# idonahum/photoVerse

Hardware: AMD Instinct MI355X
Metric: denoising steps/sec at 512x512 bs=16, 50-step loop (2 UNet fwd + CFG + DPM-Solver++ step per step) (higher is better)
Workload: dtype f16; 1 GPU; configs[1] shape timed over 96 steps instead of 50: SD-v1.5 UNet + PhotoVerse processors, 96-step loop, bs=16/GPU, 512x512 (64x64 latents), P=1, guidance 7.5, fp16; per_gpu_batch=16, global_batch=16, latent=64, parallelism=dp1 (batch-sharded, 1 all_gather), hip_graph=True, graph_branches=2

## Files before the change

photoverse_amd/csrc/pv_rowgemm.hip:

```cpp
#include "pv_common.h"
#include <stdlib.h>

namespace {

constexpr int RG_K = 320;
constexpr int RG_CHUNK = 160;
constexpr int RG_TILE = RG_CHUNK * 128;
constexpr int RG_SLOTS = 4;
constexpr int RG_SMEM = RG_SLOTS * RG_TILE;

struct pv_rowgemm_params_dev : pv_row_gemm_params {
    uint32_t w_bytes;
};

template <int N>
__device__ __forceinline__ void rg_wait_vmcnt() {
    static_assert(N >= 0 && N < 64, "vmcnt is a 6-bit field");
    asm volatile("s_waitcnt vmcnt(%0)" ::"n"(N) : "memory");
}

template <bool GEGLU>
__global__ __launch_bounds__(256, 2) void row_gemm_kernel(const pv_rowgemm_params_dev p) {
    constexpr int C = RG_K;
    constexpr int KK = C / 32;
    constexpr int KT = C / 64;
    constexpr int NFC = RG_CHUNK / 16;
    typedef unsigned uint4_t __attribute__((ext_vector_type(4)));
    typedef unsigned uint2_t __attribute__((ext_vector_type(2)));
    extern __shared__ __attribute__((aligned(16))) char smem[];

    const int lane = pv_lane_id(), wave = pv_wave_id();
    const int fr = lane & 15, g = lane >> 4;
    const int m0 = (int)blockIdx.x * 128;
    const int rows_here = min(128, p.M - m0);
    const int n_chunks = p.N / RG_CHUNK;
    const int NT = n_chunks * KT;

    const __amdgpu_buffer_rsrc_t rw = __builtin_amdgcn_make_buffer_rsrc(const_cast<void*>(p.w), 0, (int)p.w_bytes, 0x00020000);
    const __amdgpu_buffer_rsrc_t rx = __builtin_amdgcn_make_buffer_rsrc(const_cast<half_t*>(reinterpret_cast<const half_t*>(p.x)) + (size_t)m0 * p.ld_x, 0,
                                                                        rows_here * p.ld_x * 2, 0x00020000);
    const int ld_o = p.ld_out;
    const __amdgpu_buffer_rsrc_t ro = __builtin_amdgcn_make_buffer_rsrc(reinterpret_cast<half_t*>(p.out) + (size_t)m0 * ld_o, 0, rows_here * ld_o * 2, 0x00020000);

    const int lrow = lane >> 3;
    const unsigned w_lane_off = (unsigned)lrow * (unsigned)(C * 2) + (unsigned)(((lane & 7) ^ lrow) << 4);
    const unsigned piece_off = w_lane_off + (unsigned)(wave * 8) * (unsigned)(C * 2);
    auto issue_stage = [&](int t) {
        const int nc = t / KT, kt = t - nc * KT;
        char* dst = smem + (t & (RG_SLOTS - 1)) * RG_TILE;
        const int soff = nc * RG_CHUNK * (C * 2) + kt * 128;
#pragma unroll
        for (int i = 0; i < 5; ++i)
            __builtin_amdgcn_raw_ptr_buffer_load_lds(rw, PV_LDS_PTR(dst + (wave + 4 * i) * 1024), 16, (int)piece_off, soff + i * 32 * (C * 2), 0, 0);
    };
    auto wg_barrier = [&]() {
        asm volatile("s_waitcnt lgkmcnt(0)" ::: "memory");
        __builtin_amdgcn_s_barrier();
        asm volatile("" ::: "memory");
    };

    half8_t xf[KK][2];
    int mrow[2];
#pragma unroll
    for (int qi = 0; qi < 2; ++qi) {
        mrow[qi] = wave * 32 + qi * 16 + fr;
        const int off = mrow[qi] * p.ld_x * 2 + g * 16;
#pragma unroll
        for (int kk = 0; kk < KK; ++kk) xf[kk][qi] = __builtin_bit_cast(half8_t, __builtin_amdgcn_raw_buffer_load_b128(rx, off, kk * 64, 0));
    }
    issue_stage(0);
    issue_stage(1);
    if (p.x_norm) {
        const float* tab = p.x_norm + (size_t)(m0 / p.rows_per_image) * 2 * C + g * 8;
#pragma unroll
        for (int kk = 0; kk < KK; ++kk) {
            const float4_t s0 = *reinterpret_cast<const float4_t*>(tab + kk * 32), s1 = *reinterpret_cast<const float4_t*>(tab + kk * 32 + 4);
            const float4_t h0 = *reinterpret_cast<const float4_t*>(tab + C + kk * 32), h1 = *reinterpret_cast<const float4_t*>(tab + C + kk * 32 + 4);
#pragma unroll
            for (int qi = 0; qi < 2; ++qi)
#pragma unroll
                for (int j = 0; j < 8; ++j) xf[kk][qi][j] = (half_t)((float)xf[kk][qi][j] * (j < 4 ? s0[j & 3] : s1[j & 3]) + (j < 4 ? h0[j & 3] : h1[j & 3]));
        }
    }
    if (p.ln) {
        typedef _Float16 h2_t __attribute__((ext_vector_type(2)));
        const h2_t ones = h2_t{(half_t)1.0f, (half_t)1.0f};
#pragma unroll
        for (int qi = 0; qi < 2; ++qi) {
            float sum = 0.f;
#pragma unroll
            for (int kk = 0; kk < KK; ++kk)
#pragma unroll
                for (int j = 0; j < 4; ++j) sum = __builtin_amdgcn_fdot2(h2_t{xf[kk][qi][2 * j], xf[kk][qi][2 * j + 1]}, ones, sum, false);
            const float mean = pv_quad_sum(sum) * (1.0f / (float)C);
            const half_t mh = (half_t)mean;
            const h2_t nm = h2_t{(half_t)(-mh), (half_t)(-mh)};
            float sq = 0.f;
#pragma unroll
            for (int kk = 0; kk < KK; ++kk)
#pragma unroll
                for (int j = 0; j < 4; ++j) {
                    const h2_t d = h2_t{xf[kk][qi][2 * j], xf[kk][qi][2 * j + 1]} + nm;
                    sq = __builtin_amdgcn_fdot2(d, d, sq, false);
                }
            const float dm = mean - (float)mh;
            const float var = pv_quad_sum(sq) * (1.0f / (float)C) - dm * dm;
            const float rstd = rsqrtf(fmaxf(var, 0.f) + p.ln_eps);
            const float nmr = -mean * rstd;
#pragma unroll
            for (int kk = 0; kk < KK; ++kk)
#pragma unroll
                for (int j = 0; j < 8; ++j) xf[kk][qi][j] = (half_t)fmaf((float)xf[kk][qi][j], rstd, nmr);
        }
    }
    rg_wait_vmcnt<0>();

    const int ring_lane[2] = {fr * 128 + ((g ^ (fr & 7)) << 4), fr * 128 + (((4 + g) ^ (fr & 7)) << 4)};
    const int pcol = (g & 1) ? 16 + (g - 1) * 4 : g * 4;
    constexpr int OUT_PER_CHUNK = GEGLU ? RG_CHUNK / 2 : RG_CHUNK;
    constexpr int STORES = GEGLU ? 6 : 10;

    float4_t acc[NFC][2];
    for (int it = 0; it < n_chunks / 2; ++it) {
        const int t0 = it * (2 * KT);
#pragma unroll
        for (int j = 0; j < 2 * KT; ++j) {
            const int t = t0 + j;
            const int kt = j % KT;
            const int nc = 2 * it + j / KT;
            if ((j & 1) == 0) {
                const bool stores_since = (j == 6) || (j == 0 && it > 0);
                if (t >= 2) {
                    if (stores_since) rg_wait_vmcnt<STORES>(); else rg_wait_vmcnt<0>();
                }
                wg_barrier();
                if (t + 2 < NT) issue_stage(t + 2);
                if (t + 3 < NT) issue_stage(t + 3);
            }
            if (kt == 0) {
#pragma unroll
                for (int i = 0; i < NFC; ++i)
                    acc[i][0] = acc[i][1] = p.bias ? *reinterpret_cast<const float4_t*>(p.bias + nc * RG_CHUNK + i * 16 + g * 4) : float4_t{0.f, 0.f, 0.f, 0.f};
            }
            const char* slot = smem + (t & (RG_SLOTS - 1)) * RG_TILE;
#pragma unroll
            for (int ks = 0; ks < 2; ++ks) {
                const char* base = slot + ring_lane[ks];
#pragma unroll
                for (int i = 0; i < NFC; ++i) {
                    const half8_t a = *reinterpret_cast<const half8_t*>(base + i * 2048);
#pragma unroll
                    for (int qi = 0; qi < 2; ++qi) acc[i][qi] = __builtin_amdgcn_mfma_f32_16x16x32_f16(a, xf[2 * kt + ks][qi], acc[i][qi], 0, 0, 0);
                }
            }
            if (kt == KT - 1) {
                const int ocol0 = nc * OUT_PER_CHUNK;
#pragma unroll
                for (int qi = 0; qi < 2; ++qi) {
                    const int ooff = mrow[qi] * ld_o * 2 + ocol0 * 2;
                    unsigned pk[GEGLU ? NFC / 2 : NFC][2];
                    if (GEGLU) {
#pragma unroll
                        for (int q = 0; q < NFC / 2; ++q) {
                            const float4_t v = acc[2 * q][qi], gt = acc[2 * q + 1][qi];
                            pk[q][0] = __builtin_bit_cast(unsigned, half2_t{(half_t)(v[0] * pv_gelu_erf(gt[0])), (half_t)(v[1] * pv_gelu_erf(gt[1]))});
                            pk[q][1] = __builtin_bit_cast(unsigned, half2_t{(half_t)(v[2] * pv_gelu_erf(gt[2])), (half_t)(v[3] * pv_gelu_erf(gt[3]))});
                        }
                    } else {
#pragma unroll
                        for (int i = 0; i < NFC; ++i) {
                            const float4_t v = acc[i][qi];
                            pk[i][0] = __builtin_bit_cast(unsigned, half2_t{(half_t)v[0], (half_t)v[1]});
                            pk[i][1] = __builtin_bit_cast(unsigned, half2_t{(half_t)v[2], (half_t)v[3]});
                        }
                    }
                    constexpr int NOUT = GEGLU ? NFC / 2 : NFC;
#pragma unroll
                    for (int q = 0; q < NOUT / 2; ++q) {
                        const auto v0 = __builtin_amdgcn_permlane16_swap(pk[2 * q][0], pk[2 * q + 1][0], false, false);
                        const auto v1 = __builtin_amdgcn_permlane16_swap(pk[2 * q][1], pk[2 * q + 1][1], false, false);
                        const unsigned sa0 = v0[0], sb0 = v0[1], sa1 = v1[0], sb1 = v1[1];
                        __builtin_amdgcn_raw_buffer_store_b128(uint4_t{sa0, sa1, sb0, sb1}, ro, ooff + pcol * 2 + q * 64, 0, 0);
                        asm volatile("s_nop 1" ::: "memory");
                    }
                    if (NOUT & 1)
                        __builtin_amdgcn_raw_buffer_store_b64(uint2_t{pk[NOUT - 1][0], pk[NOUT - 1][1]}, ro, ooff + g * 8 + (NOUT - 1) * 32, 0, 0);
                }
                __builtin_amdgcn_sched_barrier(0);
            }
        }
    }
}

}

extern "C" int pv_row_gemm(const pv_row_gemm_params* pp, void* stream) {
    pv_rowgemm_params_dev p;
    static_cast<pv_row_gemm_params&>(p) = *pp;
    if (!p.x || !p.w || !p.out || p.M <= 0 || p.K != RG_K || p.N <= 0 || (p.N % (2 * RG_CHUNK)) || (p.ld_x % 8) || (p.ld_out % 8) || p.ld_x < RG_K ||
        p.ld_out < (p.geglu ? p.N / 2 : p.N) || (p.x_norm && (p.ln || p.rows_per_image <= 0 || (p.rows_per_image % 128) || (p.M % p.rows_per_image))))
        return (int)hipErrorInvalidValue;
    if ((size_t)p.N * RG_K * 2 >= (1ull << 31)) return (int)hipErrorInvalidValue;
    p.w_bytes = (uint32_t)p.N * RG_K * 2;
    static bool attr_set_dev[64][2] = {};
    int dev_id = 0;
    (void)hipGetDevice(&dev_id);
    bool& attr_set = attr_set_dev[dev_id & 63][p.geglu ? 1 : 0];
    auto kern = p.geglu ? row_gemm_kernel<true> : row_gemm_kernel<false>;
    if (!attr_set) {
        hipError_t e = hipFuncSetAttribute(reinterpret_cast<const void*>(kern), hipFuncAttributeMaxDynamicSharedMemorySize, RG_SMEM);
        if (e != hipSuccess) return (int)e;
        attr_set = true;
    }
    hipLaunchKernelGGL(kern, dim3((unsigned)((p.M + 127) / 128)), dim3(256), RG_SMEM, (hipStream_t)stream, p);
    return PV_CHECK_LAUNCH();
}
```

Baseline: 33.31 denoising steps/s (bs=16 per GPU, summed over GPUs).

## Split row-GEMM N-chunk into two row groups and interleave epilogue with MFMA stages

Restructures the row GEMM pipeline so each 160-column weight chunk is split into a 96-row and a 64-row group, streamed through a 6-slot LDS ring in stage pairs. The epilogue (GELU/pack/store) of one group is spread across the MFMA stages of the other group using sched_group_barrier pacing, so the stores and transcendental work overlap matrix math. Bias loads move to buffer loads issued ahead of use, and the vmcnt waits are recomputed per stage. This hides epilogue and store latency, at the cost of much more complex scheduling code and the risk of wrong vmcnt accounting or extra register pressure.

```diff
diff --git a/photoverse_amd/csrc/pv_rowgemm.hip b/photoverse_amd/csrc/pv_rowgemm.hip
--- a/photoverse_amd/csrc/pv_rowgemm.hip
+++ b/photoverse_amd/csrc/pv_rowgemm.hip
@@ -1,13 +1,16 @@
 #include "pv_common.h"
 #include <stdlib.h>
+#include <type_traits>
 
 namespace {
 
 constexpr int RG_K = 320;
 constexpr int RG_CHUNK = 160;
-constexpr int RG_TILE = RG_CHUNK * 128;
-constexpr int RG_SLOTS = 4;
-constexpr int RG_SMEM = RG_SLOTS * RG_TILE;
+constexpr int RG_ROWS_A = 96;
+constexpr int RG_SLOT = RG_ROWS_A * 128;
+constexpr int RG_SLOTS = 6;
+constexpr int RG_PAIRS = 5;
+constexpr int RG_SMEM = RG_SLOTS * RG_SLOT;
 
 struct pv_rowgemm_params_dev : pv_row_gemm_params {
     uint32_t w_bytes;
@@ -25,6 +28,7 @@
     constexpr int KK = C / 32;
     constexpr int KT = C / 64;
     constexpr int NFC = RG_CHUNK / 16;
+    constexpr int NFA = RG_ROWS_A / 16, NFB = NFC - NFA;
     typedef unsigned uint4_t __attribute__((ext_vector_type(4)));
     typedef unsigned uint2_t __attribute__((ext_vector_type(2)));
     extern __shared__ __attribute__((aligned(16))) char smem[];
@@ -34,24 +38,28 @@
     const int m0 = (int)blockIdx.x * 128;
     const int rows_here = min(128, p.M - m0);
     const int n_chunks = p.N / RG_CHUNK;
-    const int NT = n_chunks * KT;
 
     const __amdgpu_buffer_rsrc_t rw = __builtin_amdgcn_make_buffer_rsrc(const_cast<void*>(p.w), 0, (int)p.w_bytes, 0x00020000);
     const __amdgpu_buffer_rsrc_t rx = __builtin_amdgcn_make_buffer_rsrc(const_cast<half_t*>(reinterpret_cast<const half_t*>(p.x)) + (size_t)m0 * p.ld_x, 0,
                                                                         rows_here * p.ld_x * 2, 0x00020000);
+    const __amdgpu_buffer_rsrc_t rb = __builtin_amdgcn_make_buffer_rsrc(const_cast<float*>(p.bias), 0, p.bias ? p.N * 4 : 0, 0x00020000);
     const int ld_o = p.ld_out;
     const __amdgpu_buffer_rsrc_t ro = __builtin_amdgcn_make_buffer_rsrc(reinterpret_cast<half_t*>(p.out) + (size_t)m0 * ld_o, 0, rows_here * ld_o * 2, 0x00020000);
 
     const int lrow = lane >> 3;
     const unsigned w_lane_off = (unsigned)lrow * (unsigned)(C * 2) + (unsigned)(((lane & 7) ^ lrow) << 4);
     const unsigned piece_off = w_lane_off + (unsigned)(wave * 8) * (unsigned)(C * 2);
-    auto issue_stage = [&](int t) {
-        const int nc = t / KT, kt = t - nc * KT;
-        char* dst = smem + (t & (RG_SLOTS - 1)) * RG_TILE;
-        const int soff = nc * RG_CHUNK * (C * 2) + kt * 128;
-#pragma unroll
-        for (int i = 0; i < 5; ++i)
-            __builtin_amdgcn_raw_ptr_buffer_load_lds(rw, PV_LDS_PTR(dst + (wave + 4 * i) * 1024), 16, (int)piece_off, soff + i * 32 * (C * 2), 0, 0);
+    auto issue_pair = [&](int c, int pp, int sp) {
+#pragma unroll
+        for (int h = 0; h < 2; ++h) {
+            const int j = 2 * pp + h, grp = j >= KT ? 1 : 0, kt = j - grp * KT;
+            char* dst = smem + (2 * sp + h) * RG_SLOT;
+            const int soff = (c * RG_CHUNK + grp * RG_ROWS_A) * (C * 2) + kt * 128;
+#pragma unroll
+            for (int i = 0; i < 3; ++i)
+                if (i < (grp ? 2 : 3))
+                    __builtin_amdgcn_raw_ptr_buffer_load_lds(rw, PV_LDS_PTR(dst + (wave + 4 * i) * 1024), 16, (int)piece_off, soff + i * 32 * (C * 2), 0, 0);
+        }
     };
     auto wg_barrier = [&]() {
         asm volatile("s_waitcnt lgkmcnt(0)" ::: "memory");
@@ -68,8 +76,8 @@
 #pragma unroll
         for (int kk = 0; kk < KK; ++kk) xf[kk][qi] = __builtin_bit_cast(half8_t, __builtin_amdgcn_raw_buffer_load_b128(rx, off, kk * 64, 0));
     }
-    issue_stage(0);
-    issue_stage(1);
+    issue_pair(0, 0, 0);
+    issue_pair(0, 1, 1);
     if (p.x_norm) {
         const float* tab = p.x_norm + (size_t)(m0 / p.rows_per_image) * 2 * C + g * 8;
 #pragma unroll
@@ -113,83 +121,125 @@
                 for (int j = 0; j < 8; ++j) xf[kk][qi][j] = (half_t)fmaf((float)xf[kk][qi][j], rstd, nmr);
         }
     }
-    rg_wait_vmcnt<0>();
 
     const int ring_lane[2] = {fr * 128 + ((g ^ (fr & 7)) << 4), fr * 128 + (((4 + g) ^ (fr & 7)) << 4)};
     const int pcol = (g & 1) ? 16 + (g - 1) * 4 : g * 4;
     constexpr int OUT_PER_CHUNK = GEGLU ? RG_CHUNK / 2 : RG_CHUNK;
-    constexpr int STORES = GEGLU ? 6 : 10;
 
     float4_t acc[NFC][2];
-    for (int it = 0; it < n_chunks / 2; ++it) {
-        const int t0 = it * (2 * KT);
-#pragma unroll
-        for (int j = 0; j < 2 * KT; ++j) {
-            const int t = t0 + j;
-            const int kt = j % KT;
-            const int nc = 2 * it + j / KT;
-            if ((j & 1) == 0) {
-                const bool stores_since = (j == 6) || (j == 0 && it > 0);
-                if (t >= 2) {
-                    if (stores_since) rg_wait_vmcnt<STORES>(); else rg_wait_vmcnt<0>();
-                }
-                wg_barrier();
-                if (t + 2 < NT) issue_stage(t + 2);
-                if (t + 3 < NT) issue_stage(t + 3);
+    float4_t bz[NFA];
+    unsigned pk[2 * NFA];
+
+    auto load_bias = [&](int c, int fb, int nf) {
+#pragma unroll
+        for (int i = 0; i < NFA; ++i)
+            if (i < nf) bz[i] = __builtin_bit_cast(float4_t, __builtin_amdgcn_raw_buffer_load_b128(rb, g * 16, (c * RG_CHUNK + (fb + i) * 16) * 4, 0));
+    };
+
+    auto epi_word = [&](auto grp_tag, int h, int c) {
+        constexpr int GRP = decltype(grp_tag)::value, NFG = GRP ? NFB : NFA, FB = GRP ? NFA : 0;
+        constexpr int NW = GEGLU ? NFG : 2 * NFG, NOF = NW / 2;
+        const int qi = h / NW, w = h % NW, ql = w >> 1, hf = w & 1;
+        if (GEGLU) {
+            const float4_t v = acc[FB + 2 * ql][qi], gt = acc[FB + 2 * ql + 1][qi];
+            pk[w] = __builtin_bit_cast(unsigned, half2_t{(half_t)(v[2 * hf] * pv_gelu_erf(gt[2 * hf])), (half_t)(v[2 * hf + 1] * pv_gelu_erf(gt[2 * hf + 1]))});
+        } else {
+            const float4_t v = acc[FB + ql][qi];
+            pk[w] = __builtin_bit_cast(unsigned, half2_t{(half_t)v[2 * hf], (half_t)v[2 * hf + 1]});
+        }
+        if (w == NW - 1) {
+            const int ooff = mrow[qi] * ld_o * 2 + (c * OUT_PER_CHUNK + FB * (GEGLU ? 8 : 16)) * 2;
+#pragma unroll
+            for (int q = 0; q < NOF / 2; ++q) {
+                const auto v0 = __builtin_amdgcn_permlane16_swap(pk[4 * q], pk[4 * q + 2], false, false);
+                const auto v1 = __builtin_amdgcn_permlane16_swap(pk[4 * q + 1], pk[4 * q + 3], false, false);
+                const unsigned sa0 = v0[0], sb0 = v0[1], sa1 = v1[0], sb1 = v1[1];
+                __builtin_amdgcn_raw_buffer_store_b128(uint4_t{sa0, sa1, sb0, sb1}, ro, ooff + pcol * 2 + q * 64, 0, 0);
+                asm volatile("s_nop 1" ::: "memory");
             }
-            if (kt == 0) {
-#pragma unroll
-                for (int i = 0; i < NFC; ++i)
-                    acc[i][0] = acc[i][1] = p.bias ? *reinterpret_cast<const float4_t*>(p.bias + nc * RG_CHUNK + i * 16 + g * 4) : float4_t{0.f, 0.f, 0.f, 0.f};
+            if (NOF & 1) __builtin_amdgcn_raw_buffer_store_b64(uint2_t{pk[2 * (NOF - 1)], pk[2 * (NOF - 1) + 1]}, ro, ooff + g * 8 + (NOF - 1) * 32, 0, 0);
+        }
+    };
+
+    auto stage = [&](auto j_tag, auto epi_tag, int c, int sp) {
+        constexpr int j = decltype(j_tag)::value;
+        constexpr bool EPI = decltype(epi_tag)::value;
+        constexpr int GRP = j >= KT ? 1 : 0, kt = j - GRP * KT, NFG = GRP ? NFB : NFA, FB = GRP ? NFA : 0;
+        if (kt == 0) {
+#pragma unroll
+            for (int i = 0; i < NFG; ++i) acc[FB + i][0] = acc[FB + i][1] = bz[i];
+        }
+        const char* slot = smem + (2 * sp + (j & 1)) * RG_SLOT;
+#pragma unroll
+        for (int ks = 0; ks < 2; ++ks) {
+            const char* base = slot + ring_lane[ks];
+#pragma unroll
+            for (int i = 0; i < NFG; ++i) {
+                const half8_t a = *reinterpret_cast<const half8_t*>(base + i * 2048);
+#pragma unroll
+                for (int qi = 0; qi < 2; ++qi) acc[FB + i][qi] = __builtin_amdgcn_mfma_f32_16x16x32_f16(a, xf[2 * kt + ks][qi], acc[FB + i][qi], 0, 0, 0);
             }
-            const char* slot = smem + (t & (RG_SLOTS - 1)) * RG_TILE;
-#pragma unroll
-            for (int ks = 0; ks < 2; ++ks) {
-                const char* base = slot + ring_lane[ks];
-#pragma unroll
-                for (int i = 0; i < NFC; ++i) {
-                    const half8_t a = *reinterpret_cast<const half8_t*>(base + i * 2048);
-#pragma unroll
-                    for (int qi = 0; qi < 2; ++qi) acc[i][qi] = __builtin_amdgcn_mfma_f32_16x16x32_f16(a, xf[2 * kt + ks][qi], acc[i][qi], 0, 0, 0);
-                }
-            }
-            if (kt == KT - 1) {
-                const int ocol0 = nc * OUT_PER_CHUNK;
-#pragma unroll
-                for (int qi = 0; qi < 2; ++qi) {
-                    const int ooff = mrow[qi] * ld_o * 2 + ocol0 * 2;
-                    unsigned pk[GEGLU ? NFC / 2 : NFC][2];
-                    if (GEGLU) {
-#pragma unroll
-                        for (int q = 0; q < NFC / 2; ++q) {
-                            const float4_t v = acc[2 * q][qi], gt = acc[2 * q + 1][qi];
-                            pk[q][0] = __builtin_bit_cast(unsigned, half2_t{(half_t)(v[0] * pv_gelu_erf(gt[0])), (half_t)(v[1] * pv_gelu_erf(gt[1]))});
-                            pk[q][1] = __builtin_bit_cast(unsigned, half2_t{(half_t)(v[2] * pv_gelu_erf(gt[2])), (half_t)(v[3] * pv_gelu_erf(gt[3]))});
-                        }
-                    } else {
-#pragma unroll
-                        for (int i = 0; i < NFC; ++i) {
-                            const float4_t v = acc[i][qi];
-                            pk[i][0] = __builtin_bit_cast(unsigned, half2_t{(half_t)v[0], (half_t)v[1]});
-                            pk[i][1] = __builtin_bit_cast(unsigned, half2_t{(half_t)v[2], (half_t)v[3]});
-                        }
-                    }
-                    constexpr int NOUT = GEGLU ? NFC / 2 : NFC;
-#pragma unroll
-                    for (int q = 0; q < NOUT / 2; ++q) {
-                        const auto v0 = __builtin_amdgcn_permlane16_swap(pk[2 * q][0], pk[2 * q + 1][0], false, false);
-                        const auto v1 = __builtin_amdgcn_permlane16_swap(pk[2 * q][1], pk[2 * q + 1][1], false, false);
-                        const unsigned sa0 = v0[0], sb0 = v0[1], sa1 = v1[0], sb1 = v1[1];
-                        __builtin_amdgcn_raw_buffer_store_b128(uint4_t{sa0, sa1, sb0, sb1}, ro, ooff + pcol * 2 + q * 64, 0, 0);
-                        asm volatile("s_nop 1" ::: "memory");
-                    }
-                    if (NOUT & 1)
-                        __builtin_amdgcn_raw_buffer_store_b64(uint2_t{pk[NOUT - 1][0], pk[NOUT - 1][1]}, ro, ooff + g * 8 + (NOUT - 1) * 32, 0, 0);
-                }
-                __builtin_amdgcn_sched_barrier(0);
-            }
-        }
-    }
+        }
+        constexpr int NM = 4 * NFG;
+        constexpr int NFO = GRP ? NFA : NFB, H = 2 * (GEGLU ? NFO : 2 * NFO);
+        constexpr int lo = kt * H / KT, hi = (kt + 1) * H / KT;
+        static_assert(2 * H / KT <= H / 2 - 1 && H / 2 - 1 < 3 * H / KT && 4 * H / KT <= H - 1, "epilogue stores must fall into stages 2 and 4");
+        if (EPI) {
+            const int ce = GRP ? c : c - 1;
+#pragma unroll
+            for (int h = lo; h < hi; ++h) epi_word(std::integral_constant<int, 1 - GRP>{}, h, ce);
+        }
+        constexpr bool PACE_VALU = EPI && GEGLU;
+        constexpr int NT = PACE_VALU ? 4 * (hi - lo) : 0;
+        constexpr int NV = (kt == 0 ? 8 * NFG : 0) + (PACE_VALU ? 19 * (hi - lo) + 8 : 0);
+        static_assert(NT <= NM, "at most one transcendental per MFMA");
+        __builtin_amdgcn_sched_group_barrier(0x100, NFG, 0);
+#pragma unroll
+        for (int m = 0; m < NM; ++m) {
+            if (NV) __builtin_amdgcn_sched_group_barrier(0x002, (NV + NM - 1) / NM, 0);
+            if ((m + 1) * NT / NM != m * NT / NM) __builtin_amdgcn_sched_group_barrier(0x400, 1, 0);
+            __builtin_amdgcn_sched_group_barrier(0x008, 1, 0);
+            if (m < 2 * NFG && (m & 1)) __builtin_amdgcn_sched_group_barrier(0x100, 1, 0);
+        }
+        __builtin_amdgcn_sched_barrier(0);
+    };
+
+    int sp = 0;
+    auto step = [&](auto pp_tag, auto first_tag, int c) {
+        constexpr int pp = decltype(pp_tag)::value;
+        constexpr bool FIRST = decltype(first_tag)::value;
+        constexpr int SA = GEGLU ? 2 : 3, SB = GEGLU ? 1 : 2;
+        constexpr int ST[RG_PAIRS] = {0, FIRST ? 0 : SB, FIRST ? 0 : SB, SA, SA};
+        constexpr int LD[RG_PAIRS] = {6, 6, 5, 4, 4};
+        constexpr int S = pp == 0 ? 2 * SA : pp == 1 ? SA + ST[0] : ST[pp - 2] + ST[pp - 1];
+        constexpr int L = LD[(pp + 1) % RG_PAIRS];
+        if (!(FIRST && pp == 0)) {
+            if (pp == RG_PAIRS - 1 && c + 1 >= n_chunks) rg_wait_vmcnt<S>(); else rg_wait_vmcnt<S + L>();
+        }
+        if (pp == 2) load_bias(c, NFA, NFB);
+        if (pp == RG_PAIRS - 1) load_bias(min(c + 1, n_chunks - 1), 0, NFA);
+        wg_barrier();
+        const int sp2 = sp == 0 ? 2 : sp - 1;
+        if (pp + 2 < RG_PAIRS) issue_pair(c, pp + 2, sp2);
+        else if (c + 1 < n_chunks) issue_pair(c + 1, pp + 2 - RG_PAIRS, sp2);
+        stage(std::integral_constant<int, 2 * pp>{}, std::integral_constant<bool, !(FIRST && 2 * pp < KT)>{}, c, sp);
+        stage(std::integral_constant<int, 2 * pp + 1>{}, std::integral_constant<bool, !(FIRST && 2 * pp + 1 < KT)>{}, c, sp);
+        sp = sp == 2 ? 0 : sp + 1;
+    };
+    auto chunk = [&](auto first_tag, int c) {
+        step(std::integral_constant<int, 0>{}, first_tag, c);
+        step(std::integral_constant<int, 1>{}, first_tag, c);
+        step(std::integral_constant<int, 2>{}, first_tag, c);
+        step(std::integral_constant<int, 3>{}, first_tag, c);
+        step(std::integral_constant<int, 4>{}, first_tag, c);
+    };
+
+    load_bias(0, 0, NFA);
+    rg_wait_vmcnt<0>();
+    chunk(std::true_type{}, 0);
+    for (int c = 1; c < n_chunks; ++c) chunk(std::false_type{}, c);
+#pragma unroll
+    for (int h = 0; h < 2 * (GEGLU ? NFB : 2 * NFB); ++h) epi_word(std::integral_constant<int, 1>{}, h, n_chunks - 1);
 }
 
 }
```

Measured after the change: 33.53 denoising steps/s (bs=16 per GPU, summed over GPUs), median of 6. No clear change (+0.7%).
